# francesco-cal98/multimodal-idbn

Measured on AMD Instinct MI355X. Metric: CD-1 updates/sec (batch 64, 10000<->1500 RBM), higher is better.
Workload: dtype f32; 1 GPU; BASELINE configs[1] layer 1: RBM 10000<->1500 train_epoch, CD-1, batch 64 per GPU, fp32 master weights, lr 0.1 wd 1e-4 mom 0.5; global_batch=64, parallelism=dp1, arithmetic=bf16x3 split MFMA (fp32-exact products)

## Files before the change

include/imdbn_engine.h:

```cpp
#ifndef IMDBN_ENGINE_H
#define IMDBN_ENGINE_H

#include <stddef.h>
#include <stdint.h>

#ifdef __cplusplus
extern "C" {
#endif

#define IMDBN_ABI_VERSION 4

#define IMDBN_E_INVALID   (-1)
#define IMDBN_E_WORKSPACE (-2)
#define IMDBN_E_RNG       (-3)
#define IMDBN_E_NODEVICE  (-4)
#define IMDBN_E_UNSUPPORTED (-5)

#define IMDBN_PARITY_F32 0
#define IMDBN_FAST_BF16  1

#define IMDBN_RNG_PHILOX 0
#define IMDBN_RNG_REPLAY 1

#define IMDBN_MAX_GROUPS 4
// ... 70 lines not shown
int    imdbn_set_option(const char* name, int value);
typedef struct imdbn_options imdbn_options;
imdbn_options* imdbn_options_create(void);
void   imdbn_options_destroy(imdbn_options* o);
int    imdbn_options_set(imdbn_options* o, const char* name, int value);
int    imdbn_use_options(const imdbn_options* o);
int    imdbn_profile_enable(int on);
int    imdbn_profile_read(double* total_ms, int* launches);
int    imdbn_debug_stamps(long long* out, int n);
int    imdbn_debug_ws_offset(int V, int H, int B, const char* name, size_t* offset);
enum { IMDBN_ROUTE_UP_FUSED = 0, IMDBN_ROUTE_UP_STREAM_BITS = 1, IMDBN_ROUTE_UP_STREAM_REAL = 2, IMDBN_ROUTE_UP_PARTIAL4 = 3,
       IMDBN_ROUTE_UP_PARTIAL = 4 };
enum { IMDBN_ROUTE_DOWN_K2_STREAM = 0, IMDBN_ROUTE_DOWN_FUSED = 1, IMDBN_ROUTE_DOWN_CHUNKS2 = 2, IMDBN_ROUTE_DOWN_CHUNKS4 = 3,
       IMDBN_ROUTE_DOWN_TILED = 4 };
int    imdbn_debug_last_route(int route[5]);
enum { IMDBN_UPDATE_GENERIC = 0, IMDBN_UPDATE_PLANES = 1, IMDBN_UPDATE_BIN = 2, IMDBN_UPDATE_RANKS = 3 };
int    imdbn_debug_last_update(int rec[2]);

int imdbn_rng_advance(uint64_t* dev_offset, uint64_t n, imdbn_stream_t stream);

int imdbn_rbm_prop_up(const imdbn_rbm_desc* d, const float* v, int64_t ldv, int B, float T,
                      imdbn_rng* rng, float* out_prob, int64_t ldo, float* out_sample, int64_t lds,
                      void* ws, size_t ws_bytes, imdbn_stream_t stream);

int imdbn_rbm_forward(const imdbn_rbm_desc* d, const float* v, int64_t ldv, int B, int data_binary,
                      float* out_prob, int64_t ldo, void* ws, size_t ws_bytes, imdbn_stream_t stream);

int imdbn_rbm_free_energy(const imdbn_rbm_desc* d, const float* v, int64_t ldv, int B, float* out_F,
                          void* ws, size_t ws_bytes, imdbn_stream_t stream);

// ... 186 lines not shown
```

multimodal-idbn_amd/csrc/engine.hip:

```cpp
#include <hip/hip_runtime.h>

#include <algorithm>
#include <atomic>
#include <climits>
#include <cstdarg>
#include <cstdio>
#include <cstring>
#include <dlfcn.h>
#include <mutex>
#include <new>
#include <vector>

#include "../../include/imdbn_engine.h"
#include "kernels_ew.hpp"
#include "kernels_gemm.hpp"
#include "kernels_chain.hpp"
#include "kernels_stream.hpp"
#include "kernels_trace.hpp"
#include "kernels_knn.hpp"
#include "kernels_energy.hpp"
#include "kernels_metrics.hpp"
#include "kernels_ais.hpp"
#include "kernels_reverse_ais.hpp"
#include "kernels_bound.hpp"
// ... 499 lines not shown
    const void* p = nullptr;
    if (!strcmp(name, "vis_bits0")) p = L.vis_bits[0]; else if (!strcmp(name, "vis_bits1")) p = L.vis_bits[1];
    else if (!strcmp(name, "hid_bits")) p = L.hid_bits; else if (!strcmp(name, "vis_tr0")) p = L.vis_tr[0];
    else if (!strcmp(name, "vis_tr1")) p = L.vis_tr[1]; else if (!strcmp(name, "hid_tr0")) p = L.hid_tr[0];
    else if (!strcmp(name, "hid_tr1")) p = L.hid_tr[1]; else if (!strcmp(name, "cs_hpos")) p = L.cs_hpos;
    else if (!strcmp(name, "cs_hneg")) p = L.cs_hneg; else if (!strcmp(name, "cs_vpos")) p = L.cs_vpos;
    else if (!strcmp(name, "cs_vneg")) p = L.cs_vneg; else if (!strcmp(name, "flags")) p = L.flags;
    else if (!strcmp(name, "partial")) p = L.partial; else if (!strcmp(name, "vis_rm1")) p = L.vis_rm[1];
    else return fail(IMDBN_E_INVALID, "debug_ws_offset: unknown buffer %s", name);
    *offset = (size_t)((const char*)p - fake);
    return 0;
}

int imdbn_debug_last_route(int route[5]) {
    if (!route) return fail(IMDBN_E_INVALID, "imdbn_debug_last_route: null buffer");
    route[0] = t_route.up; route[1] = t_route.up_general; route[2] = t_route.down; route[3] = t_route.down_general; route[4] = t_route.down_groups;
    return 0;
}

int imdbn_debug_last_update(int rec[2]) {
    if (!rec) return fail(IMDBN_E_INVALID, "imdbn_debug_last_update: null buffer");
    rec[0] = t_update.kernel; rec[1] = t_update.tpb;
    return 0;
}

int imdbn_profile_read(double* total_ms, int* launches) {
    double tot = 0.0;
    for (size_t i = 0; i + 1 < g_prof.used; i += 2) {
        HIPCHK(hipEventSynchronize(g_prof.ev[i + 1]));
        float ms = 0.f;
        HIPCHK(hipEventElapsedTime(&ms, g_prof.ev[i], g_prof.ev[i + 1]));
// ... 1321 lines not shown
```

multimodal-idbn_amd/csrc/host_layout.hpp:

```cpp
#pragma once

struct Tuning {
    int ks_up = 0, ks_down = 0;
    int no_fast_k3 = 0;
    int no_fast_k1 = 0;
    int no_fused_up = 0;
    int k4_rows = 0;
    int no_rank_loop = 0;
    int no_chain_kernel = 0;
    int no_rank_acc = 0;
    int min_rank_loop = 2;
    int no_prefetch = 0;
    int no_bits = 0;
    int down_tr = 0;
    int no_k1s = 0;
    int k1s_ks = 0;
    int no_k2s = 0;
    int k2s_tr = 0;
    int no_k1s_real = 0;
    int no_adaptive = 0;
    int k1s_lds_pad = 0;
    int no_chain_pair = 0;
    int no_down_tiled = 0;
    int no_update_bin = 0;
    int k3_tpb = 0;
    int no_down_chunks = 0;
    int k1s_force_na = 0;
};
Tuning g_defaults;
thread_local const Tuning* t_bound = nullptr;
inline const Tuning& tune() { return t_bound ? *t_bound : g_defaults; }
int g_dbg = 0;

enum OptKind { OPT_SET, OPT_FLAG, OPT_CLAMP, OPT_CHECKED };
struct Opt { const char* name; int Tuning::*knob; OptKind kind = OPT_SET; int lo = 0, hi = 0, step = 1; };
const Opt g_opts[] = {
    {"ksplit_up", &Tuning::ks_up, OPT_CLAMP, 0, INT_MAX}, {"ksplit_down", &Tuning::ks_down, OPT_CLAMP, 0, INT_MAX},
    {"k1s_ks", &Tuning::k1s_ks, OPT_CLAMP, 0, INT_MAX}, {"k1s_lds_pad", &Tuning::k1s_lds_pad, OPT_CLAMP, 0, 64 * 1024},
    {"down_rows", &Tuning::down_tr, OPT_CHECKED, 4, 32, 4}, {"k2s_rows", &Tuning::k2s_tr, OPT_CHECKED, 8, 48, 8},
    {"chain_rows", &Tuning::k4_rows, OPT_CHECKED, 0, 16, 1},
    {"generic_k3", &Tuning::no_fast_k3, OPT_FLAG}, {"generic_k1", &Tuning::no_fast_k1, OPT_FLAG}, {"no_fused_up", &Tuning::no_fused_up, OPT_FLAG},
    {"no_rank_loop", &Tuning::no_rank_loop}, {"no_rank_acc", &Tuning::no_rank_acc}, {"min_rank_loop", &Tuning::min_rank_loop},
    {"no_chain_kernel", &Tuning::no_chain_kernel}, {"no_chain_pair", &Tuning::no_chain_pair}, {"no_bits", &Tuning::no_bits},
    {"no_prefetch", &Tuning::no_prefetch}, {"no_adaptive", &Tuning::no_adaptive}, {"k1s_force_na", &Tuning::k1s_force_na},
    {"no_k1s", &Tuning::no_k1s}, {"no_k1s_real", &Tuning::no_k1s_real}, {"no_k2s", &Tuning::no_k2s},
    {"no_down_chunks", &Tuning::no_down_chunks}, {"no_down_tiled", &Tuning::no_down_tiled},
    {"no_update_bin", &Tuning::no_update_bin}, {"k3_tpb", &Tuning::k3_tpb, OPT_CLAMP, 0, 64},
};

int set_opt(Tuning& t, const char* name, int value) {
    if (!name) return fail(IMDBN_E_INVALID, "null option name");
    if (!strcmp(name, "dbg")) { g_dbg = value; return 0; }
    for (const Opt& o : g_opts) {
        if (strcmp(name, o.name)) continue;
        if (o.kind == OPT_CHECKED && value != 0 && (value < o.lo || value > o.hi || value % o.step)) {
            if (o.step > 1) return fail(IMDBN_E_INVALID, "%s must be 0 or a multiple of %d in [%d, %d]", o.name, o.step, o.lo, o.hi);
            return fail(IMDBN_E_INVALID, "%s must be in [%d, %d]", o.name, o.lo, o.hi);
        }
        t.*o.knob = o.kind == OPT_FLAG ? (value != 0) : (o.kind == OPT_CLAMP ? std::max(o.lo, std::min(value, o.hi)) : value);
        return 0;
    }
    return fail(IMDBN_E_INVALID, "unknown option %s", name);
// ... 107 lines not shown
    L.n_loss_slots = std::max(cdiv(std::max(V, H), 64) * L.P, (cdiv(V, 8) + 2) * (L.Bp / 64)) + IMDBN_MAX_GROUPS * (L.Bp / 64);
    L.loss_part = (float*)take((size_t)L.n_loss_slots * 4);
    for (int i = 0; i < 2; ++i) {
        L.vis_tr[i] = (bf16_t*)take((size_t)3 * V * L.Bp * 2);
        if (i == 1) L.fb_bytes = (off - (((size_t)3 * V * L.Bp * 2 + 255) / 256 * 256)) + ((size_t)V * L.Bp * 2 + 255) / 256 * 256 - L.fb_off;
    }
    L.flags_h = (int*)take((size_t)L.P * cdiv(L.Hpad, 64) * 4);
    for (int i = 0; i < 2; ++i) L.vis_rm[i] = (bf16_t*)take((size_t)3 * L.Bp * L.Vpad * 2);
    L.hid_rm = (bf16_t*)take((size_t)3 * L.Bp * L.Hpad * 2);
    L.ldbits = 2 * cdiv(L.Hpad, 64);
    L.hid_bits = (uint8_t*)take((size_t)L.Bp * rup(H, 64) / 8);
    for (int i = 0; i < 2; ++i) L.vis_bits[i] = (uint8_t*)take((size_t)L.Bp * rup(V, 64) / 8);
    {
        L.k1s_tiles = cdiv(H, 32);
        int ks = t.k1s_ks > 0 ? t.k1s_ks : std::max(1, (int)((double)cus / (double)(L.k1s_tiles * mb) + 0.5));
        ks = std::min(ks, std::max(1, L.Vpad / 192));
        ks = std::max(ks, cdiv(L.Vpad, K1S_MAX_KCHUNK));
        L.k1s_kchunk = rup(cdiv(L.Vpad, ks), 64);
        L.k1s_ks = cdiv(L.Vpad, L.k1s_kchunk);
    }
    const size_t pf = std::max(std::max((size_t)L.up.ks * L.Bp * H, (size_t)L.down.ks * L.Bp * V), (size_t)L.k1s_ks * L.Bp * 32 * L.k1s_tiles);
    L.partial = (float*)take(pf * 4);
    L.k1s_cnt = (int*)take((size_t)mb * L.k1s_tiles * 4);
    L.f_h = (float*)take((size_t)L.Bp * H * 4);
    L.f_vp = (float*)take((size_t)L.Bp * V * 4);
    for (int i = 0; i < 2; ++i) L.f_v[i] = (float*)take((size_t)L.Bp * V * 4);
    L.chain_recs = (ChainRec*)take(sizeof(ChainRec) * CHAIN_MAX_STEPS);
    for (int i = 0; i < 2; ++i) {
        L.pf_rm[i] = (bf16_t*)take((size_t)3 * L.Bp * L.Vpad * 2);
        L.pf_tr[i] = (bf16_t*)take((size_t)3 * V * L.Bp * 2);
        L.pf_flags[i] = (int*)take((size_t)L.P * cdiv(L.Vpad, 64) * 4);
// ... 15 lines not shown
    std::swap(L.vis_tr[0], L.pf_tr[slot - 1]);
    std::swap(L.flags, L.pf_flags[slot - 1]);
    std::swap(L.cs_vpos, L.pf_cs[slot - 1]);
    std::swap(L.vis_bits[0], L.pf_bits[slot - 1]);
}

struct OpIn { const bf16_t* rm; int terms; const int* flag; const uint8_t* bits = nullptr; int binary = 0; };
int data_operand_kind(int data_binary) { return data_binary == IMDBN_DATA_BINARY ? 2 : (data_binary == IMDBN_DATA_UNKNOWN ? 3 : 0); }

enum class Up { fused, stream_bits, stream_real, partial };
struct Route {
    bool vec4;
    bool up_fused;
    bool k1s;
    bool k1s_real;
    bool k2s;
    bool k2s_cd;
    bool vbits;
    bool neg_rm;
    bool prefetch;
    bool next_on_k1;
    bool rides;
    bool adaptive_ok;
    bool adaptive_next;
    int tpb;
    int cd_k2_blocks;

    Up up(const OpIn& in, bool logits_only) const {
        if (up_fused) return Up::fused;
        if (!k1s || logits_only) return Up::partial;
        if (in.bits && (in.binary == 1 || in.binary == 2)) return Up::stream_bits;
        return (in.rm && k1s_real && (in.binary == 0 || (in.binary == 3 && in.bits && in.flag))) ? Up::stream_real : Up::partial;
    }
    bool data_bits(int data_binary) const { return k1s && data_binary != IMDBN_DATA_REAL; }
    bool data_needs_rm(int data_binary) const { return !(k1s && data_binary == IMDBN_DATA_BINARY); }
};

Route make_route(const imdbn_rbm_desc* d, const Layout& L) {
    const Tuning& t = tune();
    Route r{};
    r.vec4 = vec4_rows(d);
    r.up_fused = L.Vpad <= 1024 && !t.no_fused_up;
    r.k1s = r.vec4 && !t.no_k1s && !r.up_fused;
    r.k1s_real = r.k1s && !t.no_k1s_real;
    r.k2s = r.vec4 && !t.no_k2s;
    r.k2s_cd = r.k2s && !t.no_bits;
    r.vbits = d->n_groups == 0 && (r.k2s_cd || L.down_tr % 8 == 0);
    r.neg_rm = !(r.vbits && r.k1s);
    r.prefetch = r.vec4 && !t.no_prefetch;
    r.next_on_k1 = r.k2s_cd && r.vbits && r.k1s;
    r.rides = !r.k2s_cd || r.next_on_k1;
    r.tpb = t.k3_tpb > 0 ? t.k3_tpb : std::max(1, cdiv(cdiv(L.H, 128) * cdiv(L.V, 128), std::max(cu_count(), 1)));
    r.adaptive_ok = L.k1s_kchunk <= 2048 && 2 * r.tpb * L.P <= 256 && cdiv(cdiv(L.V, 128), r.tpb) <= L.k1s_tiles * L.k1s_ks;
    r.adaptive_next = r.rides && !t.no_adaptive && r.k1s_real && r.adaptive_ok;
    r.cd_k2_blocks = cdiv(L.Vpad, r.k2s_cd ? L.k2s_tr : L.down_tr);
    return r;
}
```

multimodal-idbn_amd/csrc/host_prop.hpp:

```cpp
#pragma once

using K1sFn = decltype(&k1_stream<3, 0, false, false>);
struct K1sInst { int nw, na; bool rider, general; K1sFn fn; };
const K1sInst k1s_insts[] = {
    {3, 0, true, false, k1_stream<3, 0, false, true>},  {3, 0, true, true, k1_stream<3, 0, true, true>},
    {3, 0, false, false, k1_stream<3, 0, false, false>}, {3, 0, false, true, k1_stream<3, 0, true, false>},
    {3, 1, false, false, k1_stream<3, 1, false, false>}, {3, 1, false, true, k1_stream<3, 1, true, false>},
    {3, 3, false, false, k1_stream<3, 3, false, false>}, {3, 3, false, true, k1_stream<3, 3, true, false>},
    {1, 0, true, false, k1_stream<1, 0, false, true>},  {1, 0, true, true, k1_stream<1, 0, true, true>},
    {1, 0, false, false, k1_stream<1, 0, false, false>}, {1, 0, false, true, k1_stream<1, 0, true, false>},
    {1, 1, false, false, k1_stream<1, 1, false, false>}, {1, 1, false, true, k1_stream<1, 1, true, false>},
};
using K2sFn = decltype(&k2_stream<3, 1, false>);
const K2sFn k2s_insts[2][3][2] = {
    {{k2_stream<1, 1, false>, k2_stream<1, 1, true>}, {k2_stream<1, 2, false>, k2_stream<1, 2, true>}, {k2_stream<1, 3, false>, k2_stream<1, 3, true>}},
    {{k2_stream<3, 1, false>, k2_stream<3, 1, true>}, {k2_stream<3, 2, false>, k2_stream<3, 2, true>}, {k2_stream<3, 3, false>, k2_stream<3, 3, true>}}};
using DownFn = decltype(&gemm_down_fused<3, true, 0, false>);
const DownFn down_insts[2][2][4] = {
    {{gemm_down_fused<1, false, 1, true>, gemm_down_fused<1, false, 1, false>, gemm_down_fused<1, false, 3, false>, gemm_down_fused<1, false, 0, false>},
     {gemm_down_fused<1, true, 1, true>, gemm_down_fused<1, true, 1, false>, gemm_down_fused<1, true, 3, false>, gemm_down_fused<1, true, 0, false>}},
    {{gemm_down_fused<3, false, 1, true>, gemm_down_fused<3, false, 1, false>, gemm_down_fused<3, false, 3, false>, gemm_down_fused<3, false, 0, false>},
     {gemm_down_fused<3, true, 1, true>, gemm_down_fused<3, true, 1, false>, gemm_down_fused<3, true, 3, false>, gemm_down_fused<3, true, 0, false>}}};
const DownFn down_chunk_insts[2][2] = {
    {gemm_down_fused<1, true, 0, false, 2>, gemm_down_fused<1, true, 0, false, 4>},
    {gemm_down_fused<3, true, 0, false, 2>, gemm_down_fused<3, true, 0, false, 4>}};
using DownNextFn = decltype(&gemm_down_fused_next<3, false>);
const DownNextFn down_next_insts[2][2] = {
    {gemm_down_fused_next<1, false>, gemm_down_fused_next<1, true>}, {gemm_down_fused_next<3, false>, gemm_down_fused_next<3, true>}};

int kernel_attrs_ready() {
    int dev = 0;
    HIPCHK(hipGetDevice(&dev));
    std::lock_guard<std::mutex> lock(g_devices.m);
    if ((int)g_devices.attrs.size() <= dev) g_devices.attrs.resize(dev + 1, 0);
    if (g_devices.attrs[dev]) return 0;
    const auto attr = hipFuncAttributeMaxDynamicSharedMemorySize;
    for (const K1sInst& k : k1s_insts) HIPCHK(hipFuncSetAttribute((const void*)k.fn, attr, K1S_WAVES * K1S_REGION_REAL + 8 * K1S_MAX_KCHUNK + K1S_LDS_EXTRA));
    for (const auto& nw : k2s_insts) for (const auto& mt : nw) for (K2sFn fn : mt) HIPCHK(hipFuncSetAttribute((const void*)fn, attr, 160 * 1024));
    HIPCHK(hipFuncSetAttribute((const void*)knn_topk_chunk, attr, (int)knn_chunk_lds(KNN_KMAX)));
    HIPCHK(hipFuncSetAttribute((const void*)knn_topk_merge, attr, (int)knn_merge_lds(KNN_KMAX)));
    g_devices.attrs[dev] = 1;
    return 0;
}

struct RouteRec { int up = -1, up_general = 0, down = -1, down_general = 0, down_groups = 0; };
thread_local RouteRec t_route;
inline void ran_up(int family, bool general) { t_route.up = family; t_route.up_general = general; }
inline void ran_down(int family, bool general) { t_route.down = family; t_route.down_general = general; t_route.down_groups = 0; }

FinishArgs new_finish() {
    FinishArgs f;
    memset(&f, 0, sizeof(f));
    f.T = 1.0f;
    return f;
}

void common_finish(const Ctx& c, bool up, FinishArgs& f) {
    const Layout& L = c.L;
    f.partial = L.partial;
    f.ks = up ? L.up.ks : L.down.ks;
    f.B = L.B; f.Bp = L.Bp;
    f.N = up ? L.H : L.V;
// ... 53 lines not shown
        if (a.fix_ranges > L.k1s_tiles * a.ks) return fail(IMDBN_E_INVALID, "internal: k1_stream fix-up ranges");
        c.fix_slot = false;
    }
    const int na = bit_plane ? ((t.k1s_force_na && !next) ? c.nw : 0) : ((in.terms == 1 || c.nw == 1) ? 1 : 3);
    f.dbg = c.pos_phase ? ((g_dbg & 2048) ? 64 : 0) : (g_dbg & ~2048);
    hid_bits_out(c, f, 1, 32);
    if (f.op.bits && !t.no_bits) f.op.rm = nullptr, f.rm_src = 0;
    a.region = bit_plane ? K1S_RING : K1S_REGION_REAL;
    const size_t lds = (size_t)K1S_WAVES * a.region + (size_t)8 * a.kchunk + (bit_plane ? (next ? 0 : t.k1s_lds_pad) : K1S_LDS_EXTRA);
    f.lean = finish_lean(f);
    PrepArgs pz;
    memset(&pz, 0, sizeof(pz));
    const int items = next ? cdiv(std::max(next->N, next->op.ldrm), 64) : 0;
    const int pr = next ? std::min(8, cdiv(items, L.k1s_tiles)) : 0;
    if (pr > 0 && na != 0) return fail(IMDBN_E_INVALID, "internal: preparation blocks ride on the bit-plane k1_stream only");
    for (const K1sInst& k : k1s_insts) {
        if (k.nw != c.nw || k.na != na || k.rider != (pr > 0) || k.general != !f.lean) continue;
        hipLaunchKernelGGL(k.fn, dim3(L.k1s_tiles, a.ks + pr, mb), dim3(64 * K1S_WAVES), lds, c.s, a, f, next ? *next : pz);
        HIPCHK(hipGetLastError());
        ran_up(bit_plane ? IMDBN_ROUTE_UP_STREAM_BITS : IMDBN_ROUTE_UP_STREAM_REAL, k.general);
        return 0;
    }
    return fail(IMDBN_E_INVALID, "internal: no k1_stream for %d weight and %d operand terms", c.nw, na);
}

int launch_up_partial(Ctx& c, const OpIn& in, FinishArgs f) {
    const Layout& L = c.L;
    const imdbn_rbm_desc* d = c.d;
    const int mb = L.Bp / 64;
    const int64_t ats = (int64_t)L.Bp * L.Vpad;
// ... 154 lines not shown
```

multimodal-idbn_amd/csrc/kernels_stream.hpp:

```cpp
#pragma once
#include "common.hpp"
#include "kernels_ew.hpp"
#include "kernels_gemm.hpp"

namespace imdbn {

__device__ __forceinline__ void dma16(const void* g, uint32_t lds_off) {
    uint32_t keep;
    asm volatile("s_mov_b32 %0, m0\n\ts_mov_b32 m0, %2\n\ts_nop 0\n\tglobal_load_lds_dwordx4 %1, off\n\ts_mov_b32 m0, %0"
                 : "=&s"(keep) : "v"(g), "s"(__builtin_amdgcn_readfirstlane(lds_off)) : "memory");
}
__device__ __forceinline__ void dma4(const void* g, uint32_t lds_off) {
    uint32_t keep;
    asm volatile("s_mov_b32 %0, m0\n\ts_mov_b32 m0, %2\n\ts_nop 0\n\tglobal_load_lds_dword %1, off\n\ts_mov_b32 m0, %0"
                 : "=&s"(keep) : "v"(g), "s"(__builtin_amdgcn_readfirstlane(lds_off)) : "memory");
}
template <int N> __device__ __forceinline__ void wait_vmcnt() { asm volatile("s_waitcnt vmcnt(%0)" :: "i"(N) : "memory"); }

typedef __bf16 bf16x2_t __attribute__((ext_vector_type(2)));
typedef float f32x2_t __attribute__((ext_vector_type(2)));
__device__ __forceinline__ uint32_t cvt_pk_bf16(float a, float b) {
    return __builtin_bit_cast(uint32_t, __builtin_convertvector(f32x2_t{a, b}, bf16x2_t));
}
template <int NW>
// ... 35 lines not shown
constexpr int K1S_REAL = 3;

struct K1sArgs {
    const float* W; int64_t ldw; int K, N;
    const uint8_t* abits; int Bp;
    const int* aflag; int ncb, P;
    float* slabs;
    int* counters;
    int kchunk, ks;
    int amode;
    int region;
    const bf16_t* arm; int64_t arm_ts;
    bf16_t* fix_tr; int64_t fix_ts; int fix_span, fix_ranges;
};

template <int NW, int NA, bool GE, bool RIDER>
__global__ __launch_bounds__(64 * K1S_WAVES, (RIDER && !GE) ? 4 : 2) void k1_stream(const K1sArgs a, const FinishArgs fa, const PrepArgs next) {
    constexpr bool REAL = NA > 0;
    static_assert(!(RIDER && REAL), "preparation blocks ride on the bit-plane instantiation");
    extern __shared__ __attribute__((aligned(16))) char smem[];
    if (RIDER && (int)blockIdx.y >= a.ks) {
        const int nworkers = (gridDim.y - a.ks) * gridDim.x, wid = (blockIdx.y - a.ks) * gridDim.x + blockIdx.x;
        const int ntx = (max(next.N, next.op.ldrm) + 63) / 64;
        for (int it = wid; it < ntx; it += nworkers) {
            prep_item_body<8>(next, it, blockIdx.z, reinterpret_cast<bf16_t*>(smem));
            if (next.op.rm || next.adaptive) lds_barrier();
        }
        return;
    }
    const int tid = threadIdx.x, w = __builtin_amdgcn_readfirstlane(tid >> 6), l = tid & 63, n = l & 31, kg = l >> 5;
    const int tile = blockIdx.x, sl = blockIdx.y, z = blockIdx.z, ntiles = gridDim.x;
    const int n0 = tile * 32, mb = z * 64;
    const int k0 = sl * a.kchunk;
    const int k_end = min(k0 + a.kchunk, (a.K + 15) / 16 * 16);
    const int nsteps = (k_end - k0) / 16;
    const int my_steps = (nsteps - w + K1S_WAVES - 1) / K1S_WAVES;
    const int n_slots = (my_steps + 1) / 2;
    const int REGION = a.region;
    char* ring = smem + w * REGION;
    const uint8_t* abl = reinterpret_cast<const uint8_t*>(smem + K1S_WAVES * REGION);
    uint32_t* smask = reinterpret_cast<uint32_t*>(smem + K1S_WAVES * REGION + 8 * a.kchunk);
    const uint32_t ring_lds = __builtin_amdgcn_readfirstlane((uint32_t)(size_t)(__attribute__((address_space(3))) char*)ring);
    const uint32_t abl_lds = __builtin_amdgcn_readfirstlane((uint32_t)(size_t)(__attribute__((address_space(3))) char*)smem) + K1S_WAVES * REGION;

    const bool st = (fa.dbg & 64) != 0;
    const int sblk = (z * gridDim.y + sl) * ntiles + tile;
    stamp(st, sblk, 0);
    const int cb0 = k0 / 64, cb1 = min((k_end + 63) / 64, a.ncb), wd = cb1 - cb0;
    const bool adaptive = REAL && a.amode == K1S_ADAPTIVE;
    const int fix_r = sl * ntiles + tile;
    const bool fixer = REAL && adaptive && a.fix_tr && z == 0 && fix_r < a.fix_ranges;
    constexpr int NF = 2;
    const uint32_t* sfl = smask + 16;
    const bool have_bits = !REAL || a.amode != K1S_REAL;
    if (have_bits) {
        const int nrows8 = a.kchunk / 8, last_row = (a.K + 63) / 64 * 8 - 1;
        for (int q = w; q * 16 < nrows8; q += K1S_WAVES) {
            const int br = min((k0 >> 3) + 16 * q + (l >> 2), last_row);
            dma16(a.abits + (int64_t)br * a.Bp + mb + 16 * (l & 3), abl_lds + q * 1024);
        }
    }
    const int colc = min(n0 + 4 * (l & 7), a.N - 4);
    const float* wsrc = a.W + colc;
    auto issue_slot = [&](int d, int si) __attribute__((always_inline)) {
#pragma unroll
        for (int sub = 0; sub < 2; ++sub) {
            const int i = 2 * si + sub;
            if (i < my_steps) {
                const int krow = k0 + 16 * (K1S_WAVES * i + w) + (l >> 3);
#pragma unroll
                for (int h = 0; h < 2; ++h)
                    dma16(wsrc + (int64_t)min(krow + 8 * h, a.K - 1) * a.ldw, ring_lds + ((d * 2 + sub) * 2 + h) * 1024);
            }
        }
// ... 12 lines not shown
        if constexpr (REAL) {
            if (i < my_steps) {
                const int krow = k0 + 16 * (K1S_WAVES * i + w) + (l >> 3);
#pragma unroll
                for (int h = 0; h < 2; ++h)
                    dma16(wsrc + (int64_t)min(krow + 8 * h, a.K - 1) * a.ldw, ring_lds + ((i % K1S_WSTEPS) * 2 + h) * 1024);
                const int kb = min((k0 >> 4) + K1S_WAVES * i + w, nkb - 1);
#pragma unroll
                for (int mt = 0; mt < 2; ++mt)
#pragma unroll
                    for (int t = 0; t < NA; ++t)
                        dma16(abase + t * a.arm_ts + ((int64_t)kb * a.Bp + 32 * mt) * 16, aring_lds + (((i % K1S_ASTEPS) * 2 + mt) * NA + t) * 1024);
            }
        }
    };
    const bool known_real = REAL && a.amode == K1S_REAL;
    if (known_real) {
        issue_wa(0);
        issue_wa(1);
    } else {
#pragma unroll
        for (int d = 0; d < K1S_D; ++d) issue_slot(d, d);
        if (adaptive) {
            const int i0 = fixer ? fix_r * a.fix_span : 0, nitem = fixer ? min(a.fix_span, a.ncb - i0) : 1, ne = fixer ? nitem * a.P : 1;
            const int t8 = tid & 255, ie = min(t8, ne - 1);
            const uint32_t sfl_lds = abl_lds + 8 * a.kchunk + 64 + w * 256;
            dma4(a.aflag + (int64_t)(z * 8 + (t8 >> 5)) * a.ncb + min(cb0 + (tid & 31), a.ncb - 1), sfl_lds);
            dma4(a.aflag + (int64_t)(ie / nitem) * a.ncb + i0 + (ie % nitem), sfl_lds + 2048);
        }
        if (my_steps >= 2 * K1S_D) { if (adaptive) wait_vmcnt<4 * K1S_D + NF>(); else wait_vmcnt<4 * K1S_D>(); }
        else wait_vmcnt<0>();
// ... 41 lines not shown
                }
            }
        }
    }
    uint32_t mlo = 0u;
    if constexpr (REAL) {
        if (adaptive) {
            wait_vmcnt<0>();
            const unsigned long long m = __ballot(((sfl[tid & 255] & FLAG_NONBINARY) != 0u && (tid & 31) < wd) ? 1 : 0);
            if (l == 0 && w < 4) smask[w] = (uint32_t)m | (uint32_t)(m >> 32);
        }
    }
    if (!known_real) wait_vmcnt<0>();
    stamp(st, sblk, 2);
    if (st && tid == 64 * (K1S_WAVES - 1) && sblk < 4096) g_stamps[sblk * 8 + 7] = wall_clock64();
    __syncthreads();
    if constexpr (REAL) {
        if (adaptive) mlo = __builtin_amdgcn_readfirstlane(smask[0] | smask[1] | smask[2] | smask[3]);
    }
    const bool real_loop = REAL && (known_real || mlo != 0u);
    if constexpr (REAL) if (real_loop) {
        if (!known_real) {
#pragma unroll
            for (int mt = 0; mt < 2; ++mt)
#pragma unroll
                for (int i = 0; i < 16; ++i) acc[mt][i] = 0.f;
            issue_wa(0);
            issue_wa(1);
        }
        for (int i = 0; i < my_steps; ++i) {
// ... 17 lines not shown
#pragma unroll
                    for (int t = 0; t < NA; ++t)
                        at[t] = *reinterpret_cast<const uint4*>(aring + (((i % K1S_ASTEPS) * 2 + mt) * NA + t) * 1024 + n * 32 + kg * 16);
                }
#pragma unroll
                for (int ta = 0; ta < NA; ++ta)
#pragma unroll
                    for (int tw = 0; tw < NW; ++tw)
                        acc[mt] = __builtin_amdgcn_mfma_f32_32x32x16_bf16(as_frag(at[ta]), as_frag(bf[tw]), acc[mt], 0, 0, 0);
            }
            asm volatile("s_waitcnt lgkmcnt(0)" ::: "memory");
            __builtin_amdgcn_sched_barrier(0);
            issue_wa(i + 2);
        }
        wait_vmcnt<0>();
        __syncthreads();
    }

    if constexpr (REAL) {
        auto block_or = [&](int v) __attribute__((always_inline)) {
            const bool wany = __any(v) != 0;
            if (l == 0) smask[w] = wany ? 1u : 0u;
            __syncthreads();
            uint32_t r = 0u;
#pragma unroll
            for (int ww = 0; ww < K1S_WAVES; ++ww) r |= smask[ww];
            __syncthreads();
            return r != 0u;
        };
        if (fixer && block_or(sfl[512 + (tid & 255)] & FLAG_INEXACT)) {
            const int i0 = fix_r * a.fix_span, nitem = min(a.fix_span, a.ncb - i0);
            for (int it = 0; it < nitem; ++it)
                for (int zc = 0; zc < a.Bp / 64; ++zc) {
                    const int nb = (tid < 8) ? (a.aflag[(zc * 8 + tid) * a.ncb + i0 + it] & FLAG_NONBINARY) : 0;
                    if (block_or(nb)) continue;
                    for (int i = tid; i < 2 * 64 * 8; i += 64 * K1S_WAVES) {
                        const int pl = 1 + (i >> 9), c = (i >> 3) & 63, q = i & 7, col = (i0 + it) * 64 + c;
                        if (col < a.K) *reinterpret_cast<uint4*>(a.fix_tr + pl * a.fix_ts + (int64_t)col * a.Bp + zc * 64 + 8 * q) = make_uint4(0u, 0u, 0u, 0u);
                    }
                }
        }
    }

    float* red = reinterpret_cast<float*>(smem);
#pragma unroll
    for (int mt = 0; mt < 2; ++mt)
#pragma unroll
        for (int reg = 0; reg < 16; ++reg) red[(w * 64 + mt * 32 + mfma_row(reg, l)) * 32 + n] = acc[mt][reg];
    __syncthreads();
    if constexpr (!GE) {
        auto sync8 = [&]() __attribute__((always_inline)) { asm volatile("s_waitcnt vmcnt(0) lgkmcnt(0)\n\ts_barrier" ::: "memory"); };
        const int c = tid & 31, hex = tid >> 5;
        float xs[4];
#pragma unroll
        for (int i = 0; i < 4; ++i) {
            const int o = (4 * hex + i) * 32 + c;
            float t = red[o];
#pragma unroll
            for (int ww = 1; ww < K1S_WAVES; ++ww) t += red[ww * 2048 + o];
            xs[i] = t;
        }
        int* s_words = reinterpret_cast<int*>(smem + K1S_WAVES * 8192);
        if (a.amode == K1S_ASSERTED) {
// ... 93 lines not shown
#pragma unroll
                for (int i = 0; i < 8; ++i)
                    t[q][i] = __hip_atomic_load(s0p + (int64_t)min(k + q, a.ks - 1) * ntiles * 2048 + i * 32, __ATOMIC_RELAXED, __HIP_MEMORY_SCOPE_AGENT);
#pragma unroll
            for (int q = 0; q < 8; ++q)
                if (k + q < a.ks) {
#pragma unroll
                    for (int i = 0; i < 8; ++i) xs[i] = (k + q == 0) ? __uint_as_float(t[q][i]) : xs[i] + __uint_as_float(t[q][i]);
                }
        }
    }
    stamp(st, sblk, 5);
    if (!GE || fa.lean) (void)finish_lean8(fa, ecol, mb + 8 * oct, xs, (mb >> 3) + oct, sl8, 1, 32);
    else if constexpr (GE) (void)finish_rows8(fa, ecol, mb + 8 * oct, xs, (mb >> 3) + oct, side);
    stamp(st, sblk, 6);
}


typedef __attribute__((ext_vector_type(4))) float f32x4;

constexpr int K2S_D = 3;
constexpr int K2S_W = 8;
constexpr int K2S_LW = 4;
constexpr int K2S_LDR = 68;

struct K2sArgs {
    const float* W; int64_t ldw; int K, N;
    const uint8_t* abits; int Bp;
    int TR;
};
// ... 131 lines not shown
```

multimodal-idbn_amd/imdbn/engine/hip_engine.py:

```python
from __future__ import annotations

import os
import ctypes as C
from typing import Dict, List, Optional, Sequence, Tuple

import torch

from . import native as N
from . import rng as R


def _f32c(t: torch.Tensor) -> torch.Tensor:
    if t.dtype != torch.float32:
        t = t.float()
    if t.dim() == 2 and t.stride(1) == 1 and t.stride(0) >= t.size(1):
        return t
    if not t.is_contiguous():
        t = t.contiguous()
    return t


def _ptr(t: Optional[torch.Tensor]):
    return C.c_void_p(0 if t is None else t.data_ptr())

# ... 72 lines not shown

    def profile_read(self) -> Tuple[float, int]:
        ms, n = C.c_double(0), C.c_int(0)
        self._call("imdbn_profile_read", C.byref(ms), C.byref(n))
        return ms.value, n.value

    def debug_buffer(self, dev, V, H, B, name: str, nbytes: int) -> torch.Tensor:
        off = C.c_size_t(0)
        self._call("imdbn_debug_ws_offset", int(V), int(H), int(B), name.encode(), C.byref(off))
        ws = self._workspace(torch.device(dev), V, H, B)
        return ws[off.value:off.value + nbytes]

    def last_route(self) -> dict:
        r = (C.c_int * 5)()
        self._call("imdbn_debug_last_route", r)
        return {"up": N.ROUTE_UP[r[0]] if r[0] >= 0 else None, "up_epilogue": "general" if r[1] else "lean",
                "down": N.ROUTE_DOWN[r[2]] if r[2] >= 0 else None, "down_epilogue": "general" if r[3] else "lean",
                "finish_groups": bool(r[4])}

    def _workspace(self, dev, V, H, B):
        key = (dev, V, H, B, torch.cuda.current_stream(dev).cuda_stream if torch.device(dev).type == "cuda" else 0)
        ws = self._ws.get(key)
        if ws is None:
            need = int(self._lib.imdbn_ws_bytes(V, H, B))
            ws = torch.empty(need, dtype=torch.uint8, device=dev)
            self._ws[key] = ws
        return ws

    def _ws_tail(self, dev, V, H, B):
        ws = self._workspace(dev, V, H, B)
        return _ptr(ws), ws.numel(), self._stream(dev)

    def _buffer(self, key: tuple, make, at_least: int = 0) -> torch.Tensor:
# ... 958 lines not shown
```

multimodal-idbn_amd/imdbn/engine/native.py:

```python
from __future__ import annotations

import ctypes as C
import os

MAX_GROUPS = 4
ABI_VERSION = 4
PARITY_F32, FAST_BF16 = 0, 1
RNG_PHILOX, RNG_REPLAY = 0, 1
BOUND_ENTROPY, BOUND_LOGQ = 0, 1
DELTA_UP, DELTA_DOWN = 0, 1
DATA_UNKNOWN, DATA_BINARY, DATA_REAL = 0, 1, 2
ROUTE_UP = ("fused", "stream_bits", "stream_real", "partial4", "partial")
ROUTE_DOWN = ("k2_stream", "down_fused", "down_chunks2", "down_chunks4", "down_tiled")

_HERE = os.path.dirname(os.path.abspath(__file__))
LIB_PATH = os.path.normpath(os.path.join(_HERE, "..", "..", "lib", "libimdbn_hip.so"))


class RbmDesc(C.Structure):
    _fields_ = [
        ("W", C.c_void_p), ("ldw", C.c_int64),
        ("hid_bias", C.c_void_p), ("vis_bias", C.c_void_p),
        ("W_m", C.c_void_p), ("hb_m", C.c_void_p), ("vb_m", C.c_void_p),
        ("V", C.c_int32), ("H", C.c_int32), ("mode", C.c_int32), ("n_groups", C.c_int32),
        ("group_start", C.c_int32 * MAX_GROUPS), ("group_end", C.c_int32 * MAX_GROUPS),
    ]

# ... 55 lines not shown
    "imdbn_last_error": (_INT, [C.c_char_p, _SZ]),
    "imdbn_device_info": (_INT, [C.POINTER(_INT), C.c_char_p, _SZ]),
    "imdbn_ws_bytes": (_SZ, [_INT, _INT, _INT]),
    "imdbn_set_tuning": (_INT, [_INT, _INT]),
    "imdbn_set_option": (_INT, [C.c_char_p, _INT]),
    "imdbn_options_create": (_P, []),
    "imdbn_options_destroy": (None, [_P]),
    "imdbn_options_set": (_INT, [_P, C.c_char_p, _INT]),
    "imdbn_use_options": (_INT, [_P]),
    "imdbn_profile_enable": (_INT, [_INT]),
    "imdbn_profile_read": (_INT, [C.POINTER(C.c_double), C.POINTER(_INT)]),
    "imdbn_debug_stamps": (_INT, [C.POINTER(C.c_longlong), _INT]),
    "imdbn_debug_ws_offset": (_INT, [_INT, _INT, _INT, C.c_char_p, C.POINTER(_SZ)]),
    "imdbn_debug_last_route": (_INT, [C.POINTER(_INT)]),
    "imdbn_debug_last_update": (_INT, [C.POINTER(_INT)]),
    "imdbn_rng_advance": (_INT, [_P, C.c_uint64, _P]),
    "imdbn_rbm_prop_up": (_INT, [C.POINTER(RbmDesc), _P, _I64, _INT, _F, C.POINTER(Rng), _P, _I64, _P, _I64, _P, _SZ, _P]),
    "imdbn_rbm_forward": (_INT, [C.POINTER(RbmDesc), _P, _I64, _INT, _INT, _P, _I64, _P, _SZ, _P]),
    "imdbn_rbm_free_energy": (_INT, [C.POINTER(RbmDesc), _P, _I64, _INT, _P, _P, _SZ, _P]),
    "imdbn_rbm_ais": (_INT, [C.POINTER(RbmDesc), _INT, _INT, C.POINTER(_F), _P, C.POINTER(Rng), _P, _P, _I64, _P, _SZ, _P]),
    "imdbn_rbm_ais_groups": (_INT, [C.POINTER(RbmDesc), _INT, _INT, C.POINTER(_F), _P, C.POINTER(Rng), _P, _P, _I64, _P, _SZ, _P]),
    "imdbn_rbm_reverse_ais": (_INT, [C.POINTER(RbmDesc), _P, _I64, _INT, _INT, C.POINTER(_F), _P, C.POINTER(Rng), _P, _P, _I64, _P, _SZ, _P]),
    "imdbn_rows_logmeanexp": (_INT, [_P, _INT, _INT, _P, _P, _P]),
    "imdbn_rbm_label_loglik": (_INT, [C.POINTER(RbmDesc), _P, _I64, _INT, _INT, _INT, _P, _P, _P, _P, _SZ, _P]),
    "imdbn_rbm_label_step": (_INT, [C.POINTER(RbmDesc), _P, _I64, _INT, _INT, _INT, _P, C.POINTER(CdOpts), _P, _P, _P, _SZ, _P]),
    "imdbn_rbm_pseudo_loglik": (_INT, [C.POINTER(RbmDesc), _P, _I64, _INT, _P, _P, _I64, _P, _SZ, _P]),
    "imdbn_rbm_bound_step": (_INT, [C.POINTER(RbmDesc), _P, _I64, _INT, _INT, C.POINTER(Rng), _P, _P, _I64, _P, _SZ, _P]),
    "imdbn_rbm_prop_down": (_INT, [C.POINTER(RbmDesc), _P, _I64, _INT, _F, _INT, _P, _I64, _P, _SZ, _P]),
    "imdbn_rbm_sample_visible": (_INT, [C.POINTER(RbmDesc), _P, _I64, _INT, C.POINTER(Rng), _P, _I64, _P]),
    "imdbn_rbm_gibbs_step": (_INT, [C.POINTER(RbmDesc), _P, _I64, _INT, _INT, _INT, C.POINTER(Rng), _P, _P, _P, _P, _P, _SZ, _P]),
# ... 79 lines not shown
```

Baseline: 10750 updates/s.

## Add k1_tail kernel that fuses split-K reduction into the last-arriving block

Adds a k1_tail variant of the up-pass streaming kernel for lean epilogues. Each split-K block reduces its waves' partial sums in LDS and stores them to a slab, and the last block to arrive (tracked by a counter) sums all slabs and runs the finish epilogue. The existing path does more cross-block reduction work, so this removes a synchronisation or reduction step at the cost of atomics and a serialized tail on one block per tile. It also lets an explicit k1s_ks bypass the Vpad/192 cap and guards an out-of-range bit-row DMA.

After: 10700 updates/s. About the same (-0.4%).

```diff
diff --git a/include/imdbn_engine.h b/include/imdbn_engine.h
--- a/include/imdbn_engine.h
+++ b/include/imdbn_engine.h
@@ -108,6 +108,8 @@
 enum { IMDBN_ROUTE_DOWN_K2_STREAM = 0, IMDBN_ROUTE_DOWN_FUSED = 1, IMDBN_ROUTE_DOWN_CHUNKS2 = 2, IMDBN_ROUTE_DOWN_CHUNKS4 = 3,
        IMDBN_ROUTE_DOWN_TILED = 4 };
 int    imdbn_debug_last_route(int route[5]);
+enum { IMDBN_K1_NONE = -1, IMDBN_K1_STREAM = 0, IMDBN_K1_TAIL = 1 };
+int    imdbn_debug_k1_kernel(int V, int H, int B, int operand, int na, int lean, int* kernel);
 enum { IMDBN_UPDATE_GENERIC = 0, IMDBN_UPDATE_PLANES = 1, IMDBN_UPDATE_BIN = 2, IMDBN_UPDATE_RANKS = 3 };
 int    imdbn_debug_last_update(int rec[2]);
 
diff --git a/multimodal-idbn_amd/csrc/engine.hip b/multimodal-idbn_amd/csrc/engine.hip
--- a/multimodal-idbn_amd/csrc/engine.hip
+++ b/multimodal-idbn_amd/csrc/engine.hip
@@ -537,7 +537,18 @@
 
 int imdbn_debug_last_route(int route[5]) {
     if (!route) return fail(IMDBN_E_INVALID, "imdbn_debug_last_route: null buffer");
-    route[0] = t_route.up; route[1] = t_route.up_general; route[2] = t_route.down; route[3] = t_route.down_general; route[4] = t_route.down_groups;
+    route[0] = t_route.up; route[1] = t_route.up_general | (t_route.up_tail << 1); route[2] = t_route.down; route[3] = t_route.down_general; route[4] = t_route.down_groups;
+    return 0;
+}
+
+int imdbn_debug_k1_kernel(int V, int H, int B, int operand, int na, int lean, int* kernel) {
+    if (V <= 0 || H <= 0 || B <= 0 || operand < 0 || operand > 3 || na < 0 || !kernel) return fail(IMDBN_E_INVALID, "debug_k1_kernel: bad argument");
+    imdbn_rbm_desc d;
+    memset(&d, 0, sizeof(d));
+    d.V = V; d.H = H; d.ldw = H; d.W = reinterpret_cast<float*>((uintptr_t)1 << 30);
+    const Layout L = make_layout(V, H, B, nullptr);
+    const Route r = make_route(&d, L);
+    *kernel = !r.k1s ? IMDBN_K1_NONE : (r.tail(operand, na, lean != 0) ? IMDBN_K1_TAIL : IMDBN_K1_STREAM);
     return 0;
 }
 
diff --git a/multimodal-idbn_amd/csrc/host_layout.hpp b/multimodal-idbn_amd/csrc/host_layout.hpp
--- a/multimodal-idbn_amd/csrc/host_layout.hpp
+++ b/multimodal-idbn_amd/csrc/host_layout.hpp
@@ -26,6 +26,7 @@
     int k3_tpb = 0;
     int no_down_chunks = 0;
     int k1s_force_na = 0;
+    int no_k1_tail = 0;
 };
 Tuning g_defaults;
 thread_local const Tuning* t_bound = nullptr;
@@ -45,7 +46,7 @@
     {"no_prefetch", &Tuning::no_prefetch}, {"no_adaptive", &Tuning::no_adaptive}, {"k1s_force_na", &Tuning::k1s_force_na},
     {"no_k1s", &Tuning::no_k1s}, {"no_k1s_real", &Tuning::no_k1s_real}, {"no_k2s", &Tuning::no_k2s},
     {"no_down_chunks", &Tuning::no_down_chunks}, {"no_down_tiled", &Tuning::no_down_tiled},
-    {"no_update_bin", &Tuning::no_update_bin}, {"k3_tpb", &Tuning::k3_tpb, OPT_CLAMP, 0, 64},
+    {"no_update_bin", &Tuning::no_update_bin}, {"k3_tpb", &Tuning::k3_tpb, OPT_CLAMP, 0, 64}, {"no_k1_tail", &Tuning::no_k1_tail, OPT_FLAG},
 };
 
 int set_opt(Tuning& t, const char* name, int value) {
@@ -183,7 +184,7 @@
     {
         L.k1s_tiles = cdiv(H, 32);
         int ks = t.k1s_ks > 0 ? t.k1s_ks : std::max(1, (int)((double)cus / (double)(L.k1s_tiles * mb) + 0.5));
-        ks = std::min(ks, std::max(1, L.Vpad / 192));
+        if (t.k1s_ks <= 0) ks = std::min(ks, std::max(1, L.Vpad / 192));
         ks = std::max(ks, cdiv(L.Vpad, K1S_MAX_KCHUNK));
         L.k1s_kchunk = rup(cdiv(L.Vpad, ks), 64);
         L.k1s_ks = cdiv(L.Vpad, L.k1s_kchunk);
@@ -229,6 +230,7 @@
     bool up_fused;
     bool k1s;
     bool k1s_real;
+    bool k1_tail;
     bool k2s;
     bool k2s_cd;
     bool vbits;
@@ -247,6 +249,7 @@
         if (in.bits && (in.binary == 1 || in.binary == 2)) return Up::stream_bits;
         return (in.rm && k1s_real && (in.binary == 0 || (in.binary == 3 && in.bits && in.flag))) ? Up::stream_real : Up::partial;
     }
+    bool tail(int amode, int na, bool lean) const { return k1_tail && lean && (amode == K1S_BITS ? na == 0 : (amode == K1S_ADAPTIVE && na > 0)); }
     bool data_bits(int data_binary) const { return k1s && data_binary != IMDBN_DATA_REAL; }
     bool data_needs_rm(int data_binary) const { return !(k1s && data_binary == IMDBN_DATA_BINARY); }
 };
@@ -258,6 +261,7 @@
     r.up_fused = L.Vpad <= 1024 && !t.no_fused_up;
     r.k1s = r.vec4 && !t.no_k1s && !r.up_fused;
     r.k1s_real = r.k1s && !t.no_k1s_real;
+    r.k1_tail = r.k1s && !t.no_k1_tail && L.k1s_ks > 1;
     r.k2s = r.vec4 && !t.no_k2s;
     r.k2s_cd = r.k2s && !t.no_bits;
     r.vbits = d->n_groups == 0 && (r.k2s_cd || L.down_tr % 8 == 0);
diff --git a/multimodal-idbn_amd/csrc/host_prop.hpp b/multimodal-idbn_amd/csrc/host_prop.hpp
--- a/multimodal-idbn_amd/csrc/host_prop.hpp
+++ b/multimodal-idbn_amd/csrc/host_prop.hpp
@@ -10,6 +10,11 @@
     {1, 0, true, false, k1_stream<1, 0, false, true>},  {1, 0, true, true, k1_stream<1, 0, true, true>},
     {1, 0, false, false, k1_stream<1, 0, false, false>}, {1, 0, false, true, k1_stream<1, 0, true, false>},
     {1, 1, false, false, k1_stream<1, 1, false, false>}, {1, 1, false, true, k1_stream<1, 1, true, false>},
+};
+struct K1tInst { int nw, na; bool rider; K1sFn fn; };
+const K1tInst k1t_insts[] = {
+    {3, 0, true, k1_tail<3, 0, true>}, {3, 0, false, k1_tail<3, 0, false>}, {3, 1, false, k1_tail<3, 1, false>}, {3, 3, false, k1_tail<3, 3, false>},
+    {1, 0, true, k1_tail<1, 0, true>}, {1, 0, false, k1_tail<1, 0, false>}, {1, 1, false, k1_tail<1, 1, false>},
 };
 using K2sFn = decltype(&k2_stream<3, 1, false>);
 const K2sFn k2s_insts[2][3][2] = {
@@ -36,6 +41,7 @@
     if (g_devices.attrs[dev]) return 0;
     const auto attr = hipFuncAttributeMaxDynamicSharedMemorySize;
     for (const K1sInst& k : k1s_insts) HIPCHK(hipFuncSetAttribute((const void*)k.fn, attr, K1S_WAVES * K1S_REGION_REAL + 8 * K1S_MAX_KCHUNK + K1S_LDS_EXTRA));
+    for (const K1tInst& k : k1t_insts) HIPCHK(hipFuncSetAttribute((const void*)k.fn, attr, K1S_WAVES * K1S_REGION_REAL + 8 * K1S_MAX_KCHUNK + K1S_LDS_EXTRA));
     for (const auto& nw : k2s_insts) for (const auto& mt : nw) for (K2sFn fn : mt) HIPCHK(hipFuncSetAttribute((const void*)fn, attr, 160 * 1024));
     HIPCHK(hipFuncSetAttribute((const void*)knn_topk_chunk, attr, (int)knn_chunk_lds(KNN_KMAX)));
     HIPCHK(hipFuncSetAttribute((const void*)knn_topk_merge, attr, (int)knn_merge_lds(KNN_KMAX)));
@@ -43,9 +49,9 @@
     return 0;
 }
 
-struct RouteRec { int up = -1, up_general = 0, down = -1, down_general = 0, down_groups = 0; };
+struct RouteRec { int up = -1, up_general = 0, up_tail = 0, down = -1, down_general = 0, down_groups = 0; };
 thread_local RouteRec t_route;
-inline void ran_up(int family, bool general) { t_route.up = family; t_route.up_general = general; }
+inline void ran_up(int family, bool general, bool tail = false) { t_route.up = family; t_route.up_general = general; t_route.up_tail = tail; }
 inline void ran_down(int family, bool general) { t_route.down = family; t_route.down_general = general; t_route.down_groups = 0; }
 
 FinishArgs new_finish() {
@@ -129,6 +135,16 @@
     const int items = next ? cdiv(std::max(next->N, next->op.ldrm), 64) : 0;
     const int pr = next ? std::min(8, cdiv(items, L.k1s_tiles)) : 0;
     if (pr > 0 && na != 0) return fail(IMDBN_E_INVALID, "internal: preparation blocks ride on the bit-plane k1_stream only");
+    if (c.r.tail(a.amode, na, f.lean != 0)) {
+        for (const K1tInst& k : k1t_insts) {
+            if (k.nw != c.nw || k.na != na || k.rider != (pr > 0)) continue;
+            hipLaunchKernelGGL(k.fn, dim3(L.k1s_tiles, a.ks + pr, mb), dim3(64 * K1S_WAVES), lds, c.s, a, f, next ? *next : pz);
+            HIPCHK(hipGetLastError());
+            ran_up(bit_plane ? IMDBN_ROUTE_UP_STREAM_BITS : IMDBN_ROUTE_UP_STREAM_REAL, false, true);
+            return 0;
+        }
+        return fail(IMDBN_E_INVALID, "internal: no k1_tail for %d weight and %d operand terms", c.nw, na);
+    }
     for (const K1sInst& k : k1s_insts) {
         if (k.nw != c.nw || k.na != na || k.rider != (pr > 0) || k.general != !f.lean) continue;
         hipLaunchKernelGGL(k.fn, dim3(L.k1s_tiles, a.ks + pr, mb), dim3(64 * K1S_WAVES), lds, c.s, a, f, next ? *next : pz);
diff --git a/multimodal-idbn_amd/csrc/kernels_stream.hpp b/multimodal-idbn_amd/csrc/kernels_stream.hpp
--- a/multimodal-idbn_amd/csrc/kernels_stream.hpp
+++ b/multimodal-idbn_amd/csrc/kernels_stream.hpp
@@ -73,10 +73,11 @@
     bf16_t* fix_tr; int64_t fix_ts; int fix_span, fix_ranges;
 };
 
-template <int NW, int NA, bool GE, bool RIDER>
-__global__ __launch_bounds__(64 * K1S_WAVES, (RIDER && !GE) ? 4 : 2) void k1_stream(const K1sArgs a, const FinishArgs fa, const PrepArgs next) {
+template <int NW, int NA, bool GE, bool RIDER, bool TAIL>
+__device__ __forceinline__ void k1_body(const K1sArgs& a, const FinishArgs& fa, const PrepArgs& next) {
     constexpr bool REAL = NA > 0;
     static_assert(!(RIDER && REAL), "preparation blocks ride on the bit-plane instantiation");
+    static_assert(!(TAIL && GE), "k1_tail has the lean epilogue only");
     extern __shared__ __attribute__((aligned(16))) char smem[];
     if (RIDER && (int)blockIdx.y >= a.ks) {
         const int nworkers = (gridDim.y - a.ks) * gridDim.x, wid = (blockIdx.y - a.ks) * gridDim.x + blockIdx.x;
@@ -106,17 +107,17 @@
     const int sblk = (z * gridDim.y + sl) * ntiles + tile;
     stamp(st, sblk, 0);
     const int cb0 = k0 / 64, cb1 = min((k_end + 63) / 64, a.ncb), wd = cb1 - cb0;
-    const bool adaptive = REAL && a.amode == K1S_ADAPTIVE;
+    const bool adaptive = REAL && (TAIL || a.amode == K1S_ADAPTIVE);
     const int fix_r = sl * ntiles + tile;
     const bool fixer = REAL && adaptive && a.fix_tr && z == 0 && fix_r < a.fix_ranges;
     constexpr int NF = 2;
     const uint32_t* sfl = smask + 16;
-    const bool have_bits = !REAL || a.amode != K1S_REAL;
+    const bool have_bits = TAIL || !REAL || a.amode != K1S_REAL;
     if (have_bits) {
         const int nrows8 = a.kchunk / 8, last_row = (a.K + 63) / 64 * 8 - 1;
         for (int q = w; q * 16 < nrows8; q += K1S_WAVES) {
             const int br = min((k0 >> 3) + 16 * q + (l >> 2), last_row);
-            dma16(a.abits + (int64_t)br * a.Bp + mb + 16 * (l & 3), abl_lds + q * 1024);
+            if (16 * q + (l >> 2) < nrows8) dma16(a.abits + (int64_t)br * a.Bp + mb + 16 * (l & 3), abl_lds + q * 1024);
         }
     }
     const int colc = min(n0 + 4 * (l & 7), a.N - 4);
@@ -159,7 +160,7 @@
             }
         }
     };
-    const bool known_real = REAL && a.amode == K1S_REAL;
+    const bool known_real = !TAIL && REAL && a.amode == K1S_REAL;
     if (known_real) {
         issue_wa(0);
         issue_wa(1);
@@ -231,6 +232,21 @@
     if (!known_real) wait_vmcnt<0>();
     stamp(st, sblk, 2);
     if (st && tid == 64 * (K1S_WAVES - 1) && sblk < 4096) g_stamps[sblk * 8 + 7] = wall_clock64();
+    float* red = reinterpret_cast<float*>(smem);
+    const int red_ws = TAIL ? REGION / 4 : 2048;
+    auto write_red = [&]() __attribute__((always_inline)) {
+#pragma unroll
+        for (int mt = 0; mt < 2; ++mt)
+#pragma unroll
+            for (int reg = 0; reg < 16; ++reg) red[w * red_ws + (mt * 32 + mfma_row(reg, l)) * 32 + n] = acc[mt][reg];
+    };
+    typedef __attribute__((address_space(3))) uint32_t lu32;
+    lu32* t_words = (lu32*)(smem + K1S_WAVES * REGION);
+    uint32_t t_base = 0u;
+    if constexpr (TAIL) {
+        write_red();
+        t_base = __builtin_amdgcn_readfirstlane(t_words[0]);
+    }
     __syncthreads();
     if constexpr (REAL) {
         if (adaptive) mlo = __builtin_amdgcn_readfirstlane(smask[0] | smask[1] | smask[2] | smask[3]);
@@ -278,6 +294,7 @@
             issue_wa(i + 2);
         }
         wait_vmcnt<0>();
+        if constexpr (TAIL) write_red();
         __syncthreads();
     }
 
@@ -306,11 +323,57 @@
         }
     }
 
-    float* red = reinterpret_cast<float*>(smem);
-#pragma unroll
-    for (int mt = 0; mt < 2; ++mt)
-#pragma unroll
-        for (int reg = 0; reg < 16; ++reg) red[(w * 64 + mt * 32 + mfma_row(reg, l)) * 32 + n] = acc[mt][reg];
+    if constexpr (TAIL) {
+        auto sync8 = [&]() __attribute__((always_inline)) { asm volatile("s_waitcnt vmcnt(0) lgkmcnt(0)\n\ts_barrier" ::: "memory"); };
+        const int c = tid & 31, hex = tid >> 5;
+        float xs[4];
+#pragma unroll
+        for (int i = 0; i < 4; ++i) {
+            const int o = (4 * hex + i) * 32 + c;
+            float t = red[o];
+#pragma unroll
+            for (int ww = 1; ww < K1S_WAVES; ++ww) t += red[ww * red_ws + o];
+            xs[i] = t;
+        }
+        stamp(st, sblk, 3);
+        if (a.ks > 1) {
+            typedef __attribute__((address_space(1))) uint32_t gu32;
+            gu32* mine = (gu32*)(a.slabs + (((int64_t)z * a.ks + sl) * ntiles + tile) * 2048);
+#pragma unroll
+            for (int i = 0; i < 4; ++i) __hip_atomic_store(mine + (4 * hex + i) * 32 + c, __float_as_uint(xs[i]), __ATOMIC_RELAXED, __HIP_MEMORY_SCOPE_AGENT);
+            asm volatile("s_waitcnt vmcnt(0)" ::: "memory");
+            int* cnt = a.counters + z * ntiles + tile;
+            uint32_t seen = 0u;
+            if (l == 0) seen = __hip_atomic_fetch_add(t_words, 1u, __ATOMIC_RELAXED, __HIP_MEMORY_SCOPE_WORKGROUP);
+            seen = __builtin_amdgcn_readfirstlane(seen);
+            if (seen - t_base == K1S_WAVES - 1 && l == 0)
+                t_words[1] = (__hip_atomic_fetch_add(cnt, 1, __ATOMIC_RELAXED, __HIP_MEMORY_SCOPE_AGENT) == a.ks - 1) ? 1u : 0u;
+            sync8();
+            stamp(st, sblk, 4);
+            if (!t_words[1]) return;
+            if (tid == 0) __hip_atomic_store(cnt, 0, __ATOMIC_RELAXED, __HIP_MEMORY_SCOPE_AGENT);
+            const gu32* s0p = (const gu32*)(a.slabs + ((int64_t)z * a.ks * ntiles + tile) * 2048) + (4 * hex) * 32 + c;
+            for (int k = 0; k < a.ks; k += 8) {
+                uint32_t t[8][4];
+#pragma unroll
+                for (int q = 0; q < 8; ++q)
+#pragma unroll
+                    for (int i = 0; i < 4; ++i)
+                        t[q][i] = __hip_atomic_load(s0p + (int64_t)min(k + q, a.ks - 1) * ntiles * 2048 + i * 32, __ATOMIC_RELAXED, __HIP_MEMORY_SCOPE_AGENT);
+#pragma unroll
+                for (int q = 0; q < 8; ++q)
+                    if (k + q < a.ks) {
+#pragma unroll
+                        for (int i = 0; i < 4; ++i) xs[i] = (k + q == 0) ? __uint_as_float(t[q][i]) : xs[i] + __uint_as_float(t[q][i]);
+                    }
+            }
+        }
+        stamp(st, sblk, 5);
+        finish_lean4(fa, ecol, mb + 4 * hex, xs, (mb >> 3) + (hex >> 1), sl8.bias, 1, 32);
+        stamp(st, sblk, 6);
+        return;
+    }
+    write_red();
     __syncthreads();
     if constexpr (!GE) {
         auto sync8 = [&]() __attribute__((always_inline)) { asm volatile("s_waitcnt vmcnt(0) lgkmcnt(0)\n\ts_barrier" ::: "memory"); };
@@ -434,6 +497,15 @@
     if (!GE || fa.lean) (void)finish_lean8(fa, ecol, mb + 8 * oct, xs, (mb >> 3) + oct, sl8, 1, 32);
     else if constexpr (GE) (void)finish_rows8(fa, ecol, mb + 8 * oct, xs, (mb >> 3) + oct, side);
     stamp(st, sblk, 6);
+}
+
+template <int NW, int NA, bool GE, bool RIDER>
+__global__ __launch_bounds__(64 * K1S_WAVES, (RIDER && !GE) ? 4 : 2) void k1_stream(const K1sArgs a, const FinishArgs fa, const PrepArgs next) {
+    k1_body<NW, NA, GE, RIDER, false>(a, fa, next);
+}
+template <int NW, int NA, bool RIDER>
+__global__ __launch_bounds__(64 * K1S_WAVES, RIDER ? 4 : 2) void k1_tail(const K1sArgs a, const FinishArgs fa, const PrepArgs next) {
+    k1_body<NW, NA, false, RIDER, true>(a, fa, next);
 }
 
 
diff --git a/multimodal-idbn_amd/imdbn/engine/hip_engine.py b/multimodal-idbn_amd/imdbn/engine/hip_engine.py
--- a/multimodal-idbn_amd/imdbn/engine/hip_engine.py
+++ b/multimodal-idbn_amd/imdbn/engine/hip_engine.py
@@ -110,9 +110,21 @@
     def last_route(self) -> dict:
         r = (C.c_int * 5)()
         self._call("imdbn_debug_last_route", r)
-        return {"up": N.ROUTE_UP[r[0]] if r[0] >= 0 else None, "up_epilogue": "general" if r[1] else "lean",
+        return {"up": N.ROUTE_UP[r[0]] if r[0] >= 0 else None, "up_epilogue": "general" if r[1] & 1 else "lean",
                 "down": N.ROUTE_DOWN[r[2]] if r[2] >= 0 else None, "down_epilogue": "general" if r[3] else "lean",
                 "finish_groups": bool(r[4])}
+
+    def last_up_kernel(self):
+        r = (C.c_int * 5)()
+        self._call("imdbn_debug_last_route", r)
+        if r[0] < 0 or not N.ROUTE_UP[r[0]].startswith("stream_"):
+            return None
+        return "k1_tail" if r[1] & 2 else "k1_stream"
+
+    def k1_kernel(self, V: int, H: int, B: int, operand: int, na: int, lean: bool):
+        k = C.c_int(0)
+        self._call("imdbn_debug_k1_kernel", int(V), int(H), int(B), int(operand), int(na), 1 if lean else 0, C.byref(k))
+        return {N.K1_NONE: None, N.K1_STREAM: "k1_stream", N.K1_TAIL: "k1_tail"}[k.value]
 
     def _workspace(self, dev, V, H, B):
         key = (dev, V, H, B, torch.cuda.current_stream(dev).cuda_stream if torch.device(dev).type == "cuda" else 0)
diff --git a/multimodal-idbn_amd/imdbn/engine/native.py b/multimodal-idbn_amd/imdbn/engine/native.py
--- a/multimodal-idbn_amd/imdbn/engine/native.py
+++ b/multimodal-idbn_amd/imdbn/engine/native.py
@@ -11,6 +11,8 @@
 DELTA_UP, DELTA_DOWN = 0, 1
 DATA_UNKNOWN, DATA_BINARY, DATA_REAL = 0, 1, 2
 ROUTE_UP = ("fused", "stream_bits", "stream_real", "partial4", "partial")
+K1_NONE, K1_STREAM, K1_TAIL = -1, 0, 1
+K1S_BITS, K1S_ASSERTED, K1S_ADAPTIVE, K1S_REAL = 0, 1, 2, 3
 ROUTE_DOWN = ("k2_stream", "down_fused", "down_chunks2", "down_chunks4", "down_tiled")
 
 _HERE = os.path.dirname(os.path.abspath(__file__))
@@ -96,6 +98,7 @@
     "imdbn_debug_ws_offset": (_INT, [_INT, _INT, _INT, C.c_char_p, C.POINTER(_SZ)]),
     "imdbn_debug_last_route": (_INT, [C.POINTER(_INT)]),
     "imdbn_debug_last_update": (_INT, [C.POINTER(_INT)]),
+    "imdbn_debug_k1_kernel": (_INT, [_INT, _INT, _INT, _INT, _INT, _INT, C.POINTER(_INT)]),
     "imdbn_rng_advance": (_INT, [_P, C.c_uint64, _P]),
     "imdbn_rbm_prop_up": (_INT, [C.POINTER(RbmDesc), _P, _I64, _INT, _F, C.POINTER(Rng), _P, _I64, _P, _I64, _P, _SZ, _P]),
     "imdbn_rbm_forward": (_INT, [C.POINTER(RbmDesc), _P, _I64, _INT, _INT, _P, _I64, _P, _SZ, _P]),
```
